# kibeomKim/Pytorch-DPPO

Hardware: AMD Instinct MI355X
Metric: env steps/sec (whole node), MuJoCo Humanoid-v2, 8 DPPO workers (higher is better)
Workload: dtype fp32_3xbf16; 1 GPU; model=reference actor-critic MLP (policy 376-100-100-17, value 376-500-100-1), global_batch=65536, seq_len=16, parallelism=dp1, env=Humanoid-v2, dppo_workers=1, workers_per_gpu=1, num_envs_per_gpu=4096, dist_backend=nccl, rccl_world_size=1, rollout_len=16, num_epoch=10, minibatch_rows=65536, overlap_rollout=False, per_head_kernels=True, grad_allreduce=none

## Files before the change

csrc/common.h:

```cpp
#pragma once
#include <hip/hip_runtime.h>
#include <hip/hip_fp8.h>
#include <stdint.h>

typedef __attribute__((ext_vector_type(4))) float f32x4;
typedef __attribute__((ext_vector_type(8))) __bf16 bf16x8;

#define DEV __device__ __forceinline__
typedef __attribute__((ext_vector_type(8))) float f32x8v;
DEV f32x4 ew_sub(const f32x4& a, const f32x4& b) { return a - b; }
DEV f32x8v ew_sub(const f32x8v& a, const f32x8v& b) { return a - b; }
DEV f32x8v ew_add(const f32x8v& a, const f32x8v& b) { return a + b; }
DEV f32x4 ew_mul(const f32x4& a, float s) { return a * s; }
DEV f32x4 ew_dtanh(const f32x4& a, const f32x4& h) { return a * (1.0f - h * h); }

enum { DT_F32 = 0, DT_BF16 = 1, DT_FP8 = 2, DT_S3 = 3 };

template <int DT> struct Prec;

template <> struct Prec<DT_F32> {
  using T = float;
  struct Frag { float4 lo, hi; };
  static constexpr int BYTES = 4;
  DEV static Frag load(const T* p) {
// ... 14 lines not shown
  DEV static T cvt(float x) { return x; }
  DEV static float tof(T x) { return x; }
  DEV static void put(T* b, size_t i, float x) { b[i] = x; }
  DEV static float get(const T* b, size_t i) { return b[i]; }
};

template <> struct Prec<DT_BF16> {
  using T = __bf16;
  using Frag = bf16x8;
  static constexpr int BYTES = 2;
  DEV static Frag load(const T* p) { return *reinterpret_cast<const bf16x8*>(p); }
  DEV static f32x4 mma(f32x4 c, const Frag& a, const Frag& b) {
    return __builtin_amdgcn_mfma_f32_16x16x32_bf16(a, b, c, 0, 0, 0);
  }
  DEV static T cvt(float x) { return (__bf16)x; }
  DEV static float tof(T x) { return (float)x; }
  DEV static void put(T* b, size_t i, float x) { b[i] = (__bf16)x; }
  DEV static float get(const T* b, size_t i) { return (float)b[i]; }
};

struct S3Slot { uint32_t raw; };
struct S3Frag { bf16x8 h, l; };
template <> struct Prec<DT_S3> {
  using T = S3Slot;
  using Frag = S3Frag;
  static constexpr int BYTES = 4;
  DEV static Frag load(const T* p) {
    const bf16x8* q = reinterpret_cast<const bf16x8*>(p);
    return Frag{q[0], q[1]};
  }
  DEV static f32x4 mma(f32x4 c, const Frag& a, const Frag& b) {
    c = __builtin_amdgcn_mfma_f32_16x16x32_bf16(a.l, b.h, c, 0, 0, 0);
    c = __builtin_amdgcn_mfma_f32_16x16x32_bf16(a.h, b.l, c, 0, 0, 0);
    return __builtin_amdgcn_mfma_f32_16x16x32_bf16(a.h, b.h, c, 0, 0, 0);
  }
  DEV static __bf16* hi_ptr(T* b, size_t i) { return reinterpret_cast<__bf16*>(b) + 2 * (i & ~size_t(7)) + (i & 7); }
  DEV static const __bf16* hi_ptr(const T* b, size_t i) {
    return reinterpret_cast<const __bf16*>(b) + 2 * (i & ~size_t(7)) + (i & 7);
  }
  DEV static void split(float x, __bf16& h, __bf16& l) {
    h = (__bf16)x;
    l = (__bf16)(x - (float)h);
  }
  DEV static void put(T* b, size_t i, float x) {
    __bf16* p = hi_ptr(b, i);
    split(x, p[0], p[8]);
  }
  DEV static float get(const T* b, size_t i) {
    const __bf16* p = hi_ptr(b, i);
    return (float)p[0] + (float)p[8];
  }
};
template <int DT> struct IsSplit { static constexpr bool value = DT == DT_S3; };

template <> struct Prec<DT_FP8> {
  using T = uint8_t;
  using Frag = long;
  static constexpr int BYTES = 1;
  DEV static Frag load(const T* p) { return *reinterpret_cast<const long*>(p); }
  DEV static f32x4 mma(f32x4 c, const Frag& a, const Frag& b) {
    return __builtin_amdgcn_mfma_f32_16x16x32_fp8_fp8(a, b, c, 0, 0, 0);
  }
  DEV static T cvt(float x) {
    __hip_fp8_e4m3 q(fminf(fmaxf(x, -448.f), 448.f));
    return *reinterpret_cast<uint8_t*>(&q);
  }
  DEV static float tof(T x) {
    __hip_fp8_e4m3 q;
    *reinterpret_cast<uint8_t*>(&q) = x;
    return float(q);
  }
  DEV static void put(T* b, size_t i, float x) { b[i] = cvt(x); }
  DEV static float get(const T* b, size_t i) { return tof(b[i]); }
};

__host__ __device__ inline size_t fm_index(int r, int c, int cols) {
  return ((size_t)(r >> 4) * (size_t)(cols >> 5) + (size_t)(c >> 5)) * 512u +
         (size_t)((((r & 15) + (((c & 31) >> 3) << 4)) << 3) + (c & 7));
}
__host__ __device__ inline size_t fm_frag(int rt, int ks, int cols, int lane) {
  return ((size_t)rt * (size_t)(cols >> 5) + (size_t)ks) * 512u + (size_t)lane * 8u;
}

template <typename V>
DEV void opnd_store(const V& v, V* p) {
  __builtin_nontemporal_store(v, p);
}

constexpr float Q8_SX = 64.f, Q8_SH = 256.f;
DEV uint32_t wave_umax(uint32_t v) {
#pragma unroll
  for (int o = 1; o < 64; o <<= 1) v = max(v, (uint32_t)__shfl_xor((int)v, o, 64));
  return v;
}
__host__ __device__ inline float q8_pow2(int e) {
  const uint32_t b = (uint32_t)(e + 127) << 23;
  float f;
  __builtin_memcpy(&f, &b, 4);
  return f;
}
__host__ __device__ inline int q8_exp(uint32_t amax_bits) {
  const int ex = (int)((amax_bits >> 23) & 0xffu);
  if (ex == 0 || ex == 255) return 0;
  const int e = 6 - (ex - 127);
  return e < -120 ? -120 : (e > 120 ? 120 : e);
}
DEV uint32_t q8_pack4(const f32x4& v, float s) {
  const float a = fminf(fmaxf(v[0] * s, -448.f), 448.f), b = fminf(fmaxf(v[1] * s, -448.f), 448.f);
  const float c = fminf(fmaxf(v[2] * s, -448.f), 448.f), d = fminf(fmaxf(v[3] * s, -448.f), 448.f);
  int w = __builtin_amdgcn_cvt_pk_fp8_f32(a, b, 0, false);
  return (uint32_t)__builtin_amdgcn_cvt_pk_fp8_f32(c, d, w, true);
}
DEV uint32_t q8_pack4u(const f32x4& v, float s) {
  int w = __builtin_amdgcn_cvt_pk_fp8_f32(v[0] * s, v[1] * s, 0, false);
  return (uint32_t)__builtin_amdgcn_cvt_pk_fp8_f32(v[2] * s, v[3] * s, w, true);
}
DEV float absmax4(const f32x4& v) { return fmaxf(fmaxf(fabsf(v[0]), fabsf(v[1])), fmaxf(fabsf(v[2]), fabsf(v[3]))); }

template <int DT> struct XStore { static constexpr int DTX = (DT == DT_FP8) ? DT_BF16 : DT; };

template <int DT> struct Lds {
  static constexpr int PAD = (DT == DT_FP8 ? 16 : 32) / Prec<DT>::BYTES;
  __host__ __device__ static constexpr int stride(int d) { return d + PAD; }
};

DEV float fast_tanh(float x) {
  const float e = __expf(-2.0f * fabsf(x));
  return copysignf((1.0f - e) * __builtin_amdgcn_rcpf(1.0f + e), x);
}

DEV uint32_t hash_u32(uint32_t x) {
  x ^= x >> 16; x *= 0x7FEB352Du; x ^= x >> 15; x *= 0x846CA68Bu; x ^= x >> 16;
  return x;
}
DEV uint32_t key_es(uint32_t base, uint32_t env, uint32_t step) { return hash_u32(hash_u32(env ^ base) ^ step); }
DEV uint32_t keyed(uint32_t base, uint32_t env, uint32_t step, uint32_t dim) {
  return hash_u32(key_es(base, env, step) ^ dim);
}
DEV float uniform01(uint32_t h) { return ((float)(h >> 8) + 0.5f) * (1.0f / 16777216.0f); }
DEV float2 gauss_pair(uint32_t kes, uint32_t p) {
  const float u1 = uniform01(hash_u32(kes ^ (2u * p)));
  const float u2 = uniform01(hash_u32(kes ^ (2u * p + 1u)));
  const float r = __builtin_sqrtf(-2.0f * 0.6931471805599453f * __builtin_amdgcn_logf(u1));
  return make_float2(r * __builtin_amdgcn_cosf(u2), r * __builtin_amdgcn_sinf(u2));
}
DEV float gauss(uint32_t base, uint32_t env, uint32_t step, uint32_t dim) {
  const float2 g = gauss_pair(key_es(base, env, step), dim >> 1);
  return (dim & 1u) ? g.y : g.x;
}

DEV void glds16(const void* g, void* lds) {
  __builtin_amdgcn_global_load_lds((const __attribute__((address_space(1))) void*)g,
                                   (__attribute__((address_space(3))) void*)lds, 16, 0, 0);
}

#define WAIT_VMCNT(n) __builtin_amdgcn_s_waitcnt((((n) & 15) | (7 << 4) | (15 << 8) | ((((n) >> 4) & 3) << 14)))

extern "C" void dppo_note_error(hipError_t e, const char* file, int line);

template <auto Kernel>
inline void set_max_lds_once(size_t bytes) {
  static size_t set = 0;
  if (bytes > set) {
    const hipError_t e = hipFuncSetAttribute(reinterpret_cast<const void*>(Kernel),
                                             hipFuncAttributeMaxDynamicSharedMemorySize, (int)bytes);
    if (e != hipSuccess) dppo_note_error(e, __FILE__, __LINE__);
    else set = bytes;
  }
}

#define HIP_CHECK_LAUNCH()                                          \
  do {                                                              \
    hipError_t e__ = hipGetLastError();                             \
    if (e__ != hipSuccess) dppo_note_error(e__, __FILE__, __LINE__); \
  } while (0)

__device__ __forceinline__ float slab_sum(const float* __restrict__ p, int nch, size_t st) {
  constexpr int B = 16;
  float s = 0.f;
  for (int c0 = 0; c0 < nch; c0 += B) {
    float x[B];
#pragma unroll
    for (int c = 0; c < B; ++c) x[c] = (c0 + c < nch) ? p[(size_t)(c0 + c) * st] : 0.f;
#pragma unroll
    for (int c = 0; c < B; ++c)
      if (c0 + c < nch) s += x[c];
  }
  return s;
}

__device__ __forceinline__ bool item_reduce(const float* __restrict__ part, int nprow, int npart,
                                            const int* __restrict__ red_col, int nitems, int b,
                                            float* red, float& out, int& j) {
  constexpr int RG = 256 / ITEM_IPB;
  const int tid = threadIdx.x, c = tid % ITEM_IPB, rg = tid / ITEM_IPB;
  j = ITEM_IPB * b + c;
  float s = 0.f;
  if (j < nitems && tid < 256) {
    const float* p = part + red_col[j];
    for (int r0 = rg; r0 < nprow; r0 += 16 * RG) {
      float x[16];
#pragma unroll
      for (int u = 0; u < 16; ++u) x[u] = (r0 + RG * u < nprow) ? p[(size_t)(r0 + RG * u) * npart] : 0.f;
#pragma unroll
      for (int u = 0; u < 16; ++u)
        if (r0 + RG * u < nprow) s += x[u];
    }
  }
  red[tid] = s;
  __syncthreads();
  if (tid < ITEM_IPB) {
    float o = red[tid];
#pragma unroll
    for (int g = 1; g < RG; ++g) o += red[g * ITEM_IPB + tid];
    out = o;
  }
  return tid < ITEM_IPB && j < nitems;
}
```

csrc/phead.hip:

```cpp
#include "t32.h"

namespace {

using namespace t32;

constexpr int PH_ROWS = 128;
constexpr int PH_WAVES = 4;
constexpr int PH_SB = 8 * 1024;
constexpr int PH_S = 3;
constexpr int PH_GL = 2;
constexpr int PH_XS = 3, PH_XB = 2048;
constexpr int PH_SCR = 48 * 1024;
constexpr int PH_RED = 64;
constexpr int PH_HP = 128 * 64 * 2;
constexpr int PH_DP = 128 * 32 * 2;

constexpr size_t ph_lds_bytes() {
  return (size_t)PH_S * PH_SB + PH_SCR + (PH_WAVES * PH_RED + 64) * sizeof(float);
}
static_assert(2 * ph_lds_bytes() <= 160 * 1024, "two policy workgroups per CU");
static_assert(PH_WAVES * PH_XS * PH_XB <= PH_SCR / 2 && PH_WAVES * 32 * 32 * 4 <= PH_SCR / 2 &&
              2 * PH_HP + 2 * PH_DP <= PH_SCR, "scratch: X rings | actions, then the dW staging");

DEV int ph_swz(int row) { return ((row >> 1) & 1) << 2; }

typedef __attribute__((ext_vector_type(4))) short s16x4;
DEV s16x4 tr4(const char* p) {
  s16x4 v;
  const unsigned addr = (unsigned)(size_t)(const __attribute__((address_space(3))) char*)(p);
  asm volatile("ds_read_b64_tr_b16 %0, %1" : "=v"(v) : "v"(addr));
  return v;
}
template <int DT>
DEV void ph_settle(typename VT<DT>::Frag (&fa)[2], typename VT<DT>::Frag (&fb)[2]) {
  if constexpr (DT == DT_S3) {
    asm volatile("s_waitcnt lgkmcnt(0)"
                 : "+v"(fa[0].h), "+v"(fa[0].l), "+v"(fa[1].h), "+v"(fa[1].l), "+v"(fb[0].h), "+v"(fb[0].l),
                   "+v"(fb[1].h), "+v"(fb[1].l));
  } else {
    asm volatile("s_waitcnt lgkmcnt(0)" : "+v"(fa[0]), "+v"(fa[1]), "+v"(fb[0]), "+v"(fb[1]));
  }
}
DEV bf16x8 cat8(s16x4 a0, s16x4 a1) {
  typedef __attribute__((ext_vector_type(8))) short s16x8;
  const s16x8 v{a0[0], a0[1], a0[2], a0[3], a1[0], a1[1], a1[2], a1[3]};
  return *reinterpret_cast<const bf16x8*>(&v);
}

DEV int ph_dim(int i, int h) { return (i & 3) + 8 * (i >> 2) + 4 * h; }

template <int DT, bool P2>
__global__ __launch_bounds__(PH_WAVES * 64, 2) void phead_kernel(MlpArgs a) {
  using V = VT<DT>;
  using Frag = typename V::Frag;
  constexpr bool S3 = DT == DT_S3;
  constexpr int EB = V::EB, KPS = V::KPS;
  constexpr int NS2 = S3 ? 7 : 4, NS3 = S3 ? 2 : 1, NG3 = S3 ? 2 : 1, NG2 = S3 ? 8 : 4;
  constexpr int KK2 = S3 ? 2 : 4;
  extern __shared__ __attribute__((aligned(16))) char smem[];
  const int tid = threadIdx.x, lane = tid & 63;
  const int wave = __builtin_amdgcn_readfirstlane(tid >> 6);
  const int h = lane >> 5, r = lane & 31;
  const int m0 = blockIdx.x * PH_ROWS;
  const int d0 = a.d_in[0];
  const int ns1 = (d0 >> 4) / KPS;
  const int e2 = ns1 + NS2, e3 = e2 + NS3, eg3 = e3 + NG3, ntot = eg3 + NG2;
  const int A = a.A;
  char* ring = smem;
  char* scr = smem + PH_S * PH_SB;
  char* xring = scr + wave * (PH_XS * PH_XB);
  float* red = reinterpret_cast<float*>(scr + PH_SCR);
  float* lsd = red + PH_WAVES * PH_RED;

  const int mr = m0 + 32 * wave + r;
  const bool valid = mr < a.M;
  const int rr = valid ? mr : m0;
  const int srow = a.idx ? a.idx[rr] : a.row0 + rr;
  const bool ref_loss = a.loss_kind != 0;
  float* acts = reinterpret_cast<float*>(scr + PH_SCR / 2) + wave * 32 * 32;
  {
    const float* arow = a.actions + (size_t)srow * A;
    for (int k = 0; 2 * k < A; ++k) {
      const int d = min(2 * k + h, A - 1);
      __builtin_amdgcn_global_load_lds((const __attribute__((address_space(1))) void*)(arow + d),
                                       (__attribute__((address_space(3))) void*)(acts + 64 * k), 4, 0, 0);
    }
  }
  float l_adv = a.adv[srow];
  float l_lpo = ref_loss ? 0.f : a.logp_old[srow];
  if (tid < 64) {
    const int j = tid & 31;
    lsd[tid] = tid < 32 ? (j < A ? a.log_std[j] : 0.f) : ((ref_loss && j < A) ? a.log_std_old[j] : 0.f);
  }

  const __amdgpu_buffer_rsrc_t rw = __builtin_amdgcn_make_buffer_rsrc(const_cast<void*>(a.W), (short)0, 0x7fffffff, 0x00020000);
  auto lane_off = [&](int c32, int d) __attribute__((always_inline)) -> unsigned {
    const int i = lane & 31;
    if constexpr (S3) return (unsigned)(((i >> 4) * c32 * 512 + ((i & 15) + 16 * d) * 8) * 4 + 16 * (lane >> 5));
    else return (unsigned)(((i >> 4) * c32 * 512 + ((i & 15) + 16 * (lane >> 5)) * 8) * 2);
  };
  const int c1 = d0 >> 5;
  const unsigned vo1[2] = {lane_off(c1, 0), lane_off(c1, 1)};
  const unsigned vo4[2] = {lane_off(4, 0), lane_off(4, 1)};
  const unsigned vog[2] = {lane_off(1, 0), lane_off(1, 1)};
  auto frag_u = [&](int t, int k16, int c32) __attribute__((always_inline)) {
    return t * 2 * c32 * 512 + (k16 >> 1) * 512 + (k16 & 1) * 256;
  };
  auto issue = [&](int st) __attribute__((always_inline)) {
    __attribute__((address_space(3))) char* dst =
        (__attribute__((address_space(3))) char*)(ring + (st % PH_S) * PH_SB);
#pragma unroll
    for (int i = 0; i < PH_GL; ++i) {
      const int I = PH_GL * wave + i;
      const int u = S3 ? I >> 1 : I, d = S3 ? (I & 1) : 0;
      const int tu = S3 ? u : (u & 3), ku = S3 ? 0 : (u >> 2);
      int off;
      unsigned voff;
      if (st < ns1) {
        off = a.off_w[0] + frag_u(tu, KPS * st + ku, c1);
        voff = vo1[d];
      } else if (st < e2) {
        off = a.off_w[1] + frag_u(tu, KPS * (st - ns1) + ku, 4);
        voff = vo4[d];
      } else if (st < e3) {
        off = a.off_w[2] + frag_u(0, S3 ? 4 * (st - e2) + u : u, 4);
        voff = vo4[d];
      } else if (st < eg3) {
        off = a.off_wt[2] + (S3 ? frag_u(2 * (st - e3) + (u & 1), u >> 1, 1) : frag_u(tu, ku, 1));
        voff = vog[d];
      } else {
        const int j = st - eg3, pass = j / (NG2 / 2), jj = j % (NG2 / 2);
        off = a.off_wt[1] + frag_u(2 * pass + (u & 1), KK2 * jj + (u >> 1), 4);
        voff = vo4[d];
      }
      __builtin_amdgcn_raw_ptr_buffer_load_lds(rw, dst + I * 1024, 16, voff, (unsigned)off * EB, 0, 0);
    }
  };
  const char* xrow = reinterpret_cast<const char*>(a.x_buf) + (size_t)srow * (size_t)d0 * EB;
  auto issue_x = [&](int st) __attribute__((always_inline)) {
    char* dx = xring + (st % PH_XS) * PH_XB;
#pragma unroll
    for (int e = 0; e < 2; ++e) {
      if constexpr (S3) glds16(xrow + (size_t)(16 * st + 8 * h) * 4 + 16 * e, dx + e * 1024);
      else glds16(xrow + (size_t)(16 * (2 * st + e) + 8 * h) * 2, dx + e * 1024);
    }
  };
  auto x_frag = [&](int st, int e) __attribute__((always_inline)) -> Frag {
    const char* xs = xring + (st % PH_XS) * PH_XB;
    if constexpr (S3) {
      return Frag{*reinterpret_cast<const bf16x8*>(xs + 16 * lane), *reinterpret_cast<const bf16x8*>(xs + 1024 + 16 * lane)};
    } else {
      return *reinterpret_cast<const bf16x8*>(xs + e * 1024 + 16 * lane);
    }
  };

  const __amdgpu_buffer_rsrc_t rs_x = __builtin_amdgcn_make_buffer_rsrc(a.xT, (short)0, 0x7fffffff, 0x00020000);
  const __amdgpu_buffer_rsrc_t rs_g1 = __builtin_amdgcn_make_buffer_rsrc(a.g1pT, (short)0, 0x7fffffff, 0x00020000);
  const __amdgpu_buffer_rsrc_t rs_h1 =
      __builtin_amdgcn_make_buffer_rsrc(P2 ? a.g1pT : a.h1pT, (short)0, 0x7fffffff, 0x00020000);
  const __amdgpu_buffer_rsrc_t rs_g2 =
      __builtin_amdgcn_make_buffer_rsrc(P2 ? a.g1pT : a.g2pT, (short)0, 0x7fffffff, 0x00020000);
  const unsigned vx = (unsigned)(mr * d0 + 8 * h) * EB, v128 = (unsigned)(mr * 128 + 8 * h) * EB;
  const bool write_x = a.xT_ready == 0;
  const int xst = write_x ? 2 : 0;

  asm volatile("s_waitcnt vmcnt(0)" : "+v"(l_adv), "+v"(l_lpo)::"memory");
  static_assert(PH_S == 3 && PH_XS == 3, "the wait counts below are written for 3-stage rings");
  issue_x(0);
  issue_x(1);
  issue(0);
  issue(1);

  f32x16 acc1[4], acc2[4];
#pragma unroll
  for (int t = 0; t < 4; ++t) acc1[t] = acc2[t] = f32x16{};

  auto sync = [&](int younger) __attribute__((always_inline)) {
    asm volatile("" ::: "memory");
    wait_vm_rt(younger);
    asm volatile("s_waitcnt lgkmcnt(0)" ::: "memory");
    __builtin_amdgcn_s_barrier();
    asm volatile("" ::: "memory");
  };
  VmTrack vt(ns1 == 3 ? 2 + PH_GL + xst : 2 + PH_GL + 2 * xst, xst);
  constexpr int SP = S3 ? 2 : 1;
  auto sync_t = [&](int st) __attribute__((always_inline)) {
    sync(vt.younger());
    const bool refill = st + 2 < ntot;
    if (refill) issue(st + 2);
    vt.advance(refill ? PH_GL : 0);
  };
  auto sync_late = [&](int st) __attribute__((always_inline)) {
    sync_t(st);
    return ring + (st % PH_S) * PH_SB;
  };
  auto sto = [&](__amdgpu_buffer_rsrc_t rs, unsigned vrow, unsigned fsoff, const Frag& f) __attribute__((always_inline)) {
    st_op<DT>(rs, vrow, fsoff, f);
    vt.add(SP);
  };
// ... 424 lines not shown
```

csrc/wgrad.hip:

```cpp
#include "kernels.h"
#include "mlp_core.h"

namespace {

constexpr int WG_WAVES = 8;

template <int DT>
constexpr int wgrad_frag_bytes() { return DT == DT_FP8 ? 2048 : 512 * Prec<DT>::BYTES; }
template <int DT>
constexpr int wgrad_step_rows() { return DT == DT_FP8 ? 128 : 32; }
typedef __attribute__((ext_vector_type(8))) int i32x8;

__host__ __device__ inline int wgrad_swz(int row) { return (((row >> 1) & 1) << 1) | (((row >> 3) & 1) << 2); }

DEV unsigned rm_off(int f, int sub, int lane, int FB) {
  const int li = lane & 15, g = lane >> 4;
  const int row = 8 * g + 4 * sub + (li >> 2), col = 16 * (f & 3) + 4 * (li & 3);
  return (unsigned)((f & ~3) * FB + row * 128 + (((col >> 3) ^ wgrad_swz(row)) << 4) + (col & 7) * 2);
}
__host__ __device__ inline int wgrad_swz16(int row) { return ((row & 3) << 2) | ((row >> 3) & 3); }
DEV unsigned rm_off_s3(int f, int sub, int part, int lane, int FB) {
  const int li = lane & 15, g = lane >> 4;
  const int row = 8 * g + 4 * sub + (li >> 2), col = 16 * (f & 3) + 4 * (li & 3);
  const int pos = ((col >> 3) * 2 + part) ^ wgrad_swz16(row);
  return (unsigned)((f & ~3) * FB + row * 256 + pos * 16 + (col & 7) * 2);
}
template <int DT>
DEV typename Prec<DT>::Frag rm_frag_at(const char* st, const unsigned (&o)[4]) {
  typedef __attribute__((ext_vector_type(4))) short s16x4;
  typedef __attribute__((ext_vector_type(8))) short s16x8;
  auto rd = [&](unsigned off) __attribute__((always_inline)) {
    return __builtin_amdgcn_ds_read_tr16_b64_v4i16((__attribute__((address_space(3))) s16x4*)(st + off));
  };
  auto cat = [&](s16x4 a0, s16x4 a1) __attribute__((always_inline)) {
    const s16x8 v{a0[0], a0[1], a0[2], a0[3], a1[0], a1[1], a1[2], a1[3]};
    return *reinterpret_cast<const bf16x8*>(&v);
  };
  if constexpr (IsSplit<DT>::value) {
    return S3Frag{cat(rd(o[0]), rd(o[1])), cat(rd(o[2]), rd(o[3]))};
  } else {
    return cat(rd(o[0]), rd(o[1]));
  }
}

template <int DT, int QW>
struct WgCfg {
  static constexpr int SLOTS = QW == 1 ? 24 : 40;
  static constexpr int S = DT == DT_BF16 ? 4 : (QW == 1 ? 3 : 2);
};
template <int DT, bool WIDE>
constexpr size_t wgrad_lds_bytes() {
  constexpr size_t one = (size_t)WgCfg<DT, 1>::S * WgCfg<DT, 1>::SLOTS * wgrad_frag_bytes<DT>();
  constexpr size_t two = (size_t)WgCfg<DT, 2>::S * WgCfg<DT, 2>::SLOTS * wgrad_frag_bytes<DT>();
  return WIDE && two > one ? two : one;
}
static_assert(wgrad_lds_bytes<DT_S3, true>() <= 160 * 1024 && wgrad_lds_bytes<DT_BF16, true>() <= 160 * 1024, "wgrad LDS");

template <int DT, int QW, int C>
DEV void wgrad_lds_body(const WgradArgs& a, const WgradTask& tk, char* smem) {
  using P = Prec<DT>;
  using T = typename P::T;
  using Frag = typename P::Frag;
  constexpr int FB = wgrad_frag_bytes<DT>();
  constexpr int NI = FB / 1024;
  constexpr int S = WgCfg<DT, QW>::S;
  constexpr int SB = WgCfg<DT, QW>::SLOTS * FB;
  static_assert(QW == 1 || DT == DT_S3 || DT == DT_BF16, "two quadrants per wave: split-bf16 / bf16");
  static_assert(C * WG_WAVES <= WgCfg<DT, QW>::SLOTS, "slots");
  const int tid = threadIdx.x, lane = tid & 63;
  const int wave = __builtin_amdgcn_readfirstlane(tid >> 6);
  const char* g = reinterpret_cast<const char*>(a.gT[tk.layer]);
  const char* x = reinterpret_cast<const char*>(a.xT[tk.layer]);
  const int nk = (tk.m1 - tk.m0) / wgrad_step_rows<DT>();
  const int ks0 = tk.m0 >> 5;
  const int NF = 4 * tk.nq, F = NF + 4 * tk.kq;
  const char* srcp[C][NI];
  size_t kstride[C];
  int dst[C];
#pragma unroll
  for (int q = 0; q < C; ++q) {
    const int f = wave * C + q;
    const int ff = f < F ? f : f % F;
    const bool gs = ff < NF;
    const int fl = gs ? ff : ff - NF;
    const int feat0 = (gs ? tk.n0 : tk.k0) + 16 * fl;
    const int rm = (DT == DT_S3 || DT == DT_BF16) ? (gs ? a.g_rm[tk.layer] : a.x_rm[tk.layer]) : 0;
    const char* ob = gs ? g : x;
    if (rm == 0) {
      const char* src = ob + fm_frag(feat0 >> 4, ks0, a.ld, 0) * sizeof(T);
#pragma unroll
      for (int hh = 0; hh < NI; ++hh)
        srcp[q][hh] = src + (IsSplit<DT>::value ? (size_t)hh * 1024 + (lane & 31) * 32 + (lane >> 5) * 16
                                                 : (size_t)hh * 1024 + lane * 16);
      kstride[q] = FB;
    } else {
      const int sq = fl & 3, f0 = feat0 - 16 * sq;
#pragma unroll
      for (int hh = 0; hh < NI; ++hh) {
        const int n = NI * sq + hh;
        if constexpr (IsSplit<DT>::value) {
          const int row = 4 * n + (lane >> 4);
          const int c = (lane & 15) ^ wgrad_swz16(row);
          srcp[q][hh] = ob + ((size_t)(tk.m0 + row) * rm + f0) * sizeof(T) + 16 * c;
        } else {
          const int row = 8 * n + (lane >> 3);
          const int c = (lane & 7) ^ wgrad_swz(row);
          srcp[q][hh] = ob + ((size_t)(tk.m0 + row) * rm + f0 + 8 * c) * sizeof(T);
        }
      }
      kstride[q] = (size_t)32 * rm * sizeof(T);
    }
    dst[q] = f * FB;
  }
  auto issue = [&](int k) {
    const int kk = min(k, nk - 1);
    char* st = smem + (k % S) * SB;
#pragma unroll
    for (int q = 0; q < C; ++q)
#pragma unroll
      for (int h = 0; h < NI; ++h) glds16(srcp[q][h] + (size_t)kk * kstride[q], st + dst[q] + h * 1024);
  };
  uint32_t q8v = 0;
  if constexpr (DT == DT_FP8) q8v = a.q8_rd[(a.q8_t[tk.layer] * Q8_SUB + lane) * Q8_LINE];
  const int nqw = QW == 1 ? tk.nq : tk.nq >> 1;
  const bool active = wave < nqw * tk.kq;
  constexpr bool RMOK = DT == DT_S3 || DT == DT_BF16;
  const bool g_rm = RMOK && a.g_rm[tk.layer] != 0, x_rm = RMOK && a.x_rm[tk.layer] != 0;
  const int wn = wave / tk.kq, wk = wave - (wave / tk.kq) * tk.kq;
  const unsigned fmo = IsSplit<DT>::value ? (unsigned)((lane >> 5) * 1024 + (lane & 31) * 16)
                                          : (unsigned)(lane * 8 * (int)sizeof(T));
  unsigned pat[4][4];
#pragma unroll
  for (int i = 0; i < 4; ++i) {
    pat[i][0] = pat[i][1] = pat[i][2] = pat[i][3] = 0;
    if constexpr (IsSplit<DT>::value) {
      for (int j = 0; j < 4; ++j) pat[i][j] = rm_off_s3(i, j & 1, j >> 1, lane, FB);
    } else if constexpr (RMOK) {
      pat[i][0] = rm_off(i, 0, lane, FB);
      pat[i][1] = rm_off(i, 1, lane, FB);
    }
  }
  auto frag = [&](const char* st, int slot, bool rm, int i) __attribute__((always_inline)) -> Frag {
    const char* qb = st + slot * FB;
    if constexpr (RMOK)
      if (rm) return rm_frag_at<DT>(qb, pat[i]);
    const char* b = qb + fmo + i * FB;
    if constexpr (IsSplit<DT>::value) {
      return Frag{*reinterpret_cast<const bf16x8*>(b), *reinterpret_cast<const bf16x8*>(b + 512)};
    } else {
      return P::load(reinterpret_cast<const T*>(b));
    }
  };
  f32x4 acc[QW][4][4];
#pragma unroll
  for (int u = 0; u < QW; ++u)
#pragma unroll
    for (int i = 0; i < 4; ++i)
#pragma unroll
      for (int j = 0; j < 4; ++j) acc[u][i][j] = f32x4{0.f, 0.f, 0.f, 0.f};
#pragma unroll
  for (int s = 0; s < S - 1; ++s) issue(s);
  for (int k = 0; k < nk; ++k) {
    WAIT_VMCNT(C * NI * (S - 2));
    __builtin_amdgcn_s_barrier();
    constexpr bool LATE = DT != DT_FP8;
    if (!LATE || !active) issue(k + S - 1);
    if (active) {
      const char* st = smem + (k % S) * SB;
      if constexpr (DT == DT_FP8) {
        auto rd = [&](int f) {
          const char* p = st + f * FB + lane * 8;
          const long x0 = *reinterpret_cast<const long*>(p), x1 = *reinterpret_cast<const long*>(p + 512);
          const long x2 = *reinterpret_cast<const long*>(p + 1024), x3 = *reinterpret_cast<const long*>(p + 1536);
          return i32x8{(int)x0, (int)(x0 >> 32), (int)x1, (int)(x1 >> 32), (int)x2, (int)(x2 >> 32), (int)x3,
                       (int)(x3 >> 32)};
        };
        i32x8 a8[4], b8[4];
#pragma unroll
        for (int i = 0; i < 4; ++i) {
          a8[i] = rd(wn * 4 + i);
          b8[i] = rd(NF + wk * 4 + i);
        }

#pragma unroll
        for (int i = 0; i < 4; ++i)
#pragma unroll
          for (int j = 0; j < 4; ++j)
            acc[0][i][j] = __builtin_amdgcn_mfma_scale_f32_16x16x128_f8f6f4(a8[i], b8[j], acc[0][i][j], 0, 0, 0, 127, 0, 127);
        continue;
      }
      Frag af[4], bf[4];
#pragma unroll
      for (int i = 0; i < 4; ++i) {
        af[i] = frag(st, 4 * wn, g_rm, i);
        bf[i] = frag(st, NF + 4 * wk, x_rm, i);
      }
      if constexpr (LATE) issue(k + S - 1);
#pragma unroll
      for (int i = 0; i < 4; ++i)
#pragma unroll
        for (int j = 0; j < 4; ++j) acc[0][i][j] = P::mma(acc[0][i][j], af[i], bf[j]);
      if constexpr (QW == 2) {
#pragma unroll
        for (int i = 0; i < 4; ++i) af[i] = frag(st, 4 * (wn + nqw), g_rm, i);
#pragma unroll
        for (int i = 0; i < 4; ++i)
#pragma unroll
          for (int j = 0; j < 4; ++j) acc[QW - 1][i][j] = P::mma(acc[QW - 1][i][j], af[i], bf[j]);
      }
    }
  }
  WAIT_VMCNT(0);
  if (!active) return;
  const int KE = tk.kq * 64;
  float* out = a.slab + tk.slab;
  if constexpr (DT == DT_FP8) {
    const float inv = q8_pow2(-q8_exp(wave_umax(q8v))) / a.q8_xs[tk.layer];
#pragma unroll
    for (int i = 0; i < 4; ++i)
#pragma unroll
      for (int j = 0; j < 4; ++j) acc[0][i][j] *= inv;
  }
  const int col = wk * 64 + (lane & 15);
#pragma unroll
  for (int u = 0; u < QW; ++u) {
    const int rbase = (wn + u * nqw) * 64 + (lane >> 4) * 4;
#pragma unroll
    for (int i = 0; i < 4; ++i)
#pragma unroll
      for (int j = 0; j < 4; ++j)
#pragma unroll
        for (int q = 0; q < 4; ++q) out[(rbase + 16 * i + q) * KE + col + 16 * j] = acc[u][i][j][q];
  }
}

template <int DT, bool WIDE>
__global__ __launch_bounds__(WG_WAVES * 64) void wgrad_kernel(WgradArgs a) {
  extern __shared__ __attribute__((aligned(16))) char smem[];
  const WgradTask tk = a.tasks[blockIdx.x];
  const int F = 4 * (tk.nq + tk.kq);
  if constexpr (WIDE) {
    if (tk.nq * tk.kq > WG_WAVES) {
      if (F <= 4 * WG_WAVES) wgrad_lds_body<DT, 2, 4>(a, tk, smem);
      else wgrad_lds_body<DT, 2, 5>(a, tk, smem);
      return;
    }
  }
  if (F <= 2 * WG_WAVES) wgrad_lds_body<DT, 1, 2>(a, tk, smem);
  else wgrad_lds_body<DT, 1, 3>(a, tk, smem);
}

template <int DT, bool WIDE>
void launch_wgrad_lds(const WgradArgs& a, hipStream_t s) {
  const size_t lds = wgrad_lds_bytes<DT, WIDE>();
  set_max_lds_once<wgrad_kernel<DT, WIDE>>(lds);
  hipLaunchKernelGGL((wgrad_kernel<DT, WIDE>), dim3(a.ntasks), dim3(WG_WAVES * 64), lds, s, a);
}

__global__ __launch_bounds__(256) void grad_gather_kernel(const float* __restrict__ slab,
                                                          const int* __restrict__ src_off,
                                                          const int* __restrict__ src_meta,
                                                          const float* __restrict__ part,
                                                          int nblk, int npart, const int* __restrict__ red_col,
                                                          const int* __restrict__ red_dst, int nitems,
                                                          float scale, float* __restrict__ grad, SlabRuns runs,
                                                          float* __restrict__ loss_out) {
  const int nrb = item_blocks(nitems);
  if ((int)blockIdx.x < nrb) {
    __shared__ float red[256];
    float tot = 0.f;
    int j;
    if (item_reduce(part, nblk, npart, red_col, nitems, blockIdx.x, red, tot, j)) {
      const int d = red_dst[j];
      if (d >= 0) grad[d] = tot * scale;
      else loss_out[-1 - d] = tot;
    }
    return;
  }
  const int nb = gridDim.x - nrb;
  for (int j = (blockIdx.x - nrb) * 256 + threadIdx.x; j < runs.total; j += nb * 256) {
    const int i = runs.flat(j);
    const int mt = src_meta[i];
    const int o = src_off[i];
    const int nch = mt >> 5;
    const size_t st = (size_t)(mt & 31) << 12;
    const float s = slab_sum(slab + o, nch, st);
    grad[i] = s * scale;
  }
}

}

extern "C" int wgrad_task_ok(int dt, int nq, int kq) {
  if (nq < 1 || kq < 1) return 0;
  if (nq * kq <= WG_WAVES) return nq + kq <= 6;
  return (dt == DT_S3 || dt == DT_BF16) && nq * kq <= 2 * WG_WAVES && nq % 2 == 0 && nq + kq <= 10;
}

extern "C" void launch_wgrad(int dt, const WgradArgs& a, hipStream_t s) {
  if (a.ntasks <= 0) return;
  if (dt == DT_F32) launch_wgrad_lds<DT_F32, false>(a, s);
  else if (dt == DT_FP8) launch_wgrad_lds<DT_FP8, false>(a, s);
  else if (dt == DT_S3) {
    if (a.wide) launch_wgrad_lds<DT_S3, true>(a, s);
    else launch_wgrad_lds<DT_S3, false>(a, s);
  } else {
    if (a.wide) launch_wgrad_lds<DT_BF16, true>(a, s);
    else launch_wgrad_lds<DT_BF16, false>(a, s);
  }
  HIP_CHECK_LAUNCH();
}

extern "C" void launch_grad_gather(const float* slab, const int* src_off, const int* src_meta, const float* part,
                                   int nblk, int npart, const int* red_col, const int* red_dst, int nitems,
                                   float scale, float* grad, const SlabRuns& runs, float* loss_out, hipStream_t s) {
  int grid = (runs.total + 255) / 256;
  if (grid > 2048) grid = 2048;
  if (grid < 1) grid = 1;
  grid += item_blocks(nitems);
  hipLaunchKernelGGL(grad_gather_kernel, dim3(grid), dim3(256), 0, s, slab, src_off, src_meta, part, nblk, npart,
                     red_col, red_dst, nitems, scale, grad, runs, loss_out);
  HIP_CHECK_LAUNCH();
}
```

pytorch_dppo_amd/ops/_build.py:

```python
from __future__ import annotations

import concurrent.futures as cf
import hashlib
import os
import subprocess
import sys
import sysconfig

ROOT = os.path.dirname(os.path.dirname(os.path.dirname(os.path.abspath(__file__))))
CSRC = os.path.join(ROOT, "csrc")
BUILD = os.path.join(ROOT, "build")
OUT_DIR = os.path.dirname(os.path.abspath(__file__))
EXT_NAME = "_dppo_hip"
ARCH = os.environ.get("DPPO_OFFLOAD_ARCH", "gfx950")
HIPCC = os.environ.get("HIPCC", "/opt/rocm/bin/hipcc")
DEVICE_SRCS = ["rollout.hip", "eval.hip", "mlp.hip", "mlp_head.hip", "phead.hip", "wgrad.hip", "optim.hip", "obs.hip"]
HOST_SRCS = ["bindings.cpp", "comm.cpp"]
HEADERS = ["common.h", "mlp_core.h", "kernels.h", "t32.h"]


def ext_path(variant: str = "") -> str:
    name = EXT_NAME + (f"_{variant}" if variant else "")
    return os.path.join(OUT_DIR, name + sysconfig.get_config_var("EXT_SUFFIX"))


def _torch_flags(ext_name: str = EXT_NAME):
    import torch
    from torch.utils import cpp_extension as ce
    inc = ce.include_paths(device_type="cuda")
    libdirs = ce.library_paths(device_type="cuda")
    abi = int(torch._C._GLIBCXX_USE_CXX11_ABI)
    cflags = [f"-I{p}" for p in inc] + [f"-I{sysconfig.get_paths()['include']}",
                                         f"-D_GLIBCXX_USE_CXX11_ABI={abi}",
                                         f"-DTORCH_EXTENSION_NAME={ext_name}",
                                         "-DTORCH_API_INCLUDE_EXTENSION_H", "-DUSE_ROCM=1"]
    ldflags = [f"-L{p}" for p in libdirs] + [f"-Wl,-rpath,{p}" for p in libdirs] + [
        "-lc10", "-ltorch", "-ltorch_cpu", "-ltorch_python", "-lc10_hip", "-ltorch_hip",
        "-lrccl"]
    return cflags, ldflags


def _digest(paths, extra: str) -> str:
    h = hashlib.sha256(extra.encode())
    for p in paths:
        with open(p, "rb") as f:
            h.update(f.read())
    return h.hexdigest()[:16]


def _compile(src: str, cflags, verbose: bool, csrc: str = CSRC, extra=()) -> str:
    srcp = os.path.join(csrc, src)
    deps = [srcp] + [os.path.join(csrc, h) for h in HEADERS]
    base = ["-O3", "-std=c++17", "-fPIC", f"--offload-arch={ARCH}", "-Wno-unused-result",
            "-mllvm", "-amdgpu-mfma-vgpr-form"]
    base += os.environ.get("DPPO_EXTRA_CFLAGS", "").split() + list(extra)
    flags = base + cflags
    key = _digest(deps, " ".join(flags))
    obj = os.path.join(BUILD, f"{os.path.splitext(src)[0]}-{key}.o")
    if os.path.exists(obj):
        return obj
    cmd = [HIPCC] + flags + ["-c", srcp, "-o", obj]
    if verbose:
        print(" ".join(cmd), flush=True)
    r = subprocess.run(cmd, capture_output=True, text=True)
    if r.returncode != 0:
        raise RuntimeError(f"hipcc failed for {src}:\n{r.stderr[-6000:]}")
    return obj


def build(verbose: bool = False, force: bool = False, variant: str = "", csrc: str = CSRC, defines=()) -> str:
    os.makedirs(BUILD, exist_ok=True)
    tcflags, ldflags = _torch_flags(EXT_NAME + (f"_{variant}" if variant else ""))
    jobs = [(s, []) for s in DEVICE_SRCS] + [(s, tcflags) for s in HOST_SRCS]
    with cf.ThreadPoolExecutor(max_workers=min(8, os.cpu_count() or 4)) as ex:
        extra = [f"-D{d}" for d in defines]
        objs = list(ex.map(lambda j: _compile(j[0], j[1], verbose, csrc, extra), jobs))
    out = ext_path(variant)
    key = hashlib.sha256((" ".join(os.path.basename(o) for o in objs) + " "
                          + " ".join(ldflags)).encode()).hexdigest()[:16]
    stamp = out + ".stamp"
    if not force and os.path.exists(out) and os.path.exists(stamp) and open(stamp).read() == key:
        return out
    tmp = out + ".tmp.so"
    cmd = [HIPCC, "-shared", "-fPIC", f"--offload-arch={ARCH}"] + objs + ldflags + ["-o", tmp]
    if verbose:
        print(" ".join(cmd), flush=True)
    r = subprocess.run(cmd, capture_output=True, text=True)
    if r.returncode != 0:
        raise RuntimeError(f"link failed:\n{r.stderr[-6000:]}")
    os.replace(tmp, out)
    with open(stamp, "w") as f:
        f.write(key)
    return out


if __name__ == "__main__":
    args = sys.argv[1:]
    var = args[args.index("--variant") + 1] if "--variant" in args else ""
    src = args[args.index("--src") + 1] if "--src" in args else CSRC
    defs = args[args.index("--define") + 1].split(",") if "--define" in args else []
    p = build(verbose="-v" in args, force="--force" in args, variant=var, csrc=src, defines=defs)
    print(p)
```

Before: 15.93 million env_steps/s.

## Specialize wgrad on operand layout and add half-stage LDS ring for split-bf16

The weight-gradient kernel is now instantiated per combination of row-major or feature-major operand layout, so the runtime branch inside the inner loop is gone. LDS fragment reads now use inline asm with immediate offsets, are issued before the next async global-to-LDS refill, and are drained with one explicit lgkmcnt wait. For split-bf16 with two quadrants per wave, a new five-unit half-stage ring refills half-tiles at a finer grain to deepen prefetch within the LDS budget. The rewritten addressing and wait counts add risk of ordering or correctness errors, and having more template variants increases code size.

```diff
diff --git a/csrc/common.h b/csrc/common.h
--- a/csrc/common.h
+++ b/csrc/common.h
@@ -190,6 +190,36 @@
 DEV void glds16(const void* g, void* lds) {
   __builtin_amdgcn_global_load_lds((const __attribute__((address_space(1))) void*)g,
                                    (__attribute__((address_space(3))) void*)lds, 16, 0, 0);
+}
+
+typedef __attribute__((ext_vector_type(4))) short s16x4;
+DEV unsigned lds_addr(const void* p) {
+  return (unsigned)(size_t)(const __attribute__((address_space(3))) char*)(p);
+}
+DEV s16x4 tr4(const char* p) {
+  s16x4 v;
+  const unsigned addr = lds_addr(p);
+  asm volatile("ds_read_b64_tr_b16 %0, %1" : "=v"(v) : "v"(addr));
+  return v;
+}
+template <int OFF>
+DEV s16x4 tr4_at(unsigned addr) {
+  static_assert(OFF >= 0 && OFF < 65536, "ds offset field");
+  s16x4 v;
+  asm volatile("ds_read_b64_tr_b16 %0, %1 offset:%2" : "=v"(v) : "v"(addr), "i"(OFF));
+  return v;
+}
+template <int OFF>
+DEV bf16x8 lds_rd16_at(unsigned addr) {
+  static_assert(OFF >= 0 && OFF < 65536, "ds offset field");
+  bf16x8 v;
+  asm volatile("ds_read_b128 %0, %1 offset:%2" : "=v"(v) : "v"(addr), "i"(OFF));
+  return v;
+}
+DEV bf16x8 cat8(s16x4 a0, s16x4 a1) {
+  typedef __attribute__((ext_vector_type(8))) short s16x8;
+  const s16x8 v{a0[0], a0[1], a0[2], a0[3], a1[0], a1[1], a1[2], a1[3]};
+  return *reinterpret_cast<const bf16x8*>(&v);
 }
 
 #define WAIT_VMCNT(n) __builtin_amdgcn_s_waitcnt((((n) & 15) | (7 << 4) | (15 << 8) | ((((n) >> 4) & 3) << 14)))
diff --git a/csrc/phead.hip b/csrc/phead.hip
--- a/csrc/phead.hip
+++ b/csrc/phead.hip
@@ -24,13 +24,6 @@
 
 DEV int ph_swz(int row) { return ((row >> 1) & 1) << 2; }
 
-typedef __attribute__((ext_vector_type(4))) short s16x4;
-DEV s16x4 tr4(const char* p) {
-  s16x4 v;
-  const unsigned addr = (unsigned)(size_t)(const __attribute__((address_space(3))) char*)(p);
-  asm volatile("ds_read_b64_tr_b16 %0, %1" : "=v"(v) : "v"(addr));
-  return v;
-}
 template <int DT>
 DEV void ph_settle(typename VT<DT>::Frag (&fa)[2], typename VT<DT>::Frag (&fb)[2]) {
   if constexpr (DT == DT_S3) {
@@ -40,11 +33,6 @@
   } else {
     asm volatile("s_waitcnt lgkmcnt(0)" : "+v"(fa[0]), "+v"(fa[1]), "+v"(fb[0]), "+v"(fb[1]));
   }
-}
-DEV bf16x8 cat8(s16x4 a0, s16x4 a1) {
-  typedef __attribute__((ext_vector_type(8))) short s16x8;
-  const s16x8 v{a0[0], a0[1], a0[2], a0[3], a1[0], a1[1], a1[2], a1[3]};
-  return *reinterpret_cast<const bf16x8*>(&v);
 }
 
 DEV int ph_dim(int i, int h) { return (i & 3) + 8 * (i >> 2) + 4 * h; }
diff --git a/csrc/wgrad.hip b/csrc/wgrad.hip
--- a/csrc/wgrad.hip
+++ b/csrc/wgrad.hip
@@ -1,3 +1,5 @@
+#include <type_traits>
+
 #include "kernels.h"
 #include "mlp_core.h"
 
@@ -19,44 +21,85 @@
   return (unsigned)((f & ~3) * FB + row * 128 + (((col >> 3) ^ wgrad_swz(row)) << 4) + (col & 7) * 2);
 }
 __host__ __device__ inline int wgrad_swz16(int row) { return ((row & 3) << 2) | ((row >> 3) & 3); }
-DEV unsigned rm_off_s3(int f, int sub, int part, int lane, int FB) {
+DEV unsigned rm_off_s3(int f, int sub, int part, int lane, int FB, int rmask = 31) {
   const int li = lane & 15, g = lane >> 4;
   const int row = 8 * g + 4 * sub + (li >> 2), col = 16 * (f & 3) + 4 * (li & 3);
   const int pos = ((col >> 3) * 2 + part) ^ wgrad_swz16(row);
-  return (unsigned)((f & ~3) * FB + row * 256 + pos * 16 + (col & 7) * 2);
-}
-template <int DT>
-DEV typename Prec<DT>::Frag rm_frag_at(const char* st, const unsigned (&o)[4]) {
-  typedef __attribute__((ext_vector_type(4))) short s16x4;
-  typedef __attribute__((ext_vector_type(8))) short s16x8;
-  auto rd = [&](unsigned off) __attribute__((always_inline)) {
-    return __builtin_amdgcn_ds_read_tr16_b64_v4i16((__attribute__((address_space(3))) s16x4*)(st + off));
-  };
-  auto cat = [&](s16x4 a0, s16x4 a1) __attribute__((always_inline)) {
-    const s16x8 v{a0[0], a0[1], a0[2], a0[3], a1[0], a1[1], a1[2], a1[3]};
-    return *reinterpret_cast<const bf16x8*>(&v);
-  };
+  return (unsigned)((f & ~3) * FB + (row & rmask) * 256 + pos * 16 + (col & 7) * 2);
+}
+template <int DT, bool RM>
+struct WgRaw {
+  using Piece = std::conditional_t<RM, s16x4, bf16x8>;
+  static constexpr int NP = (IsSplit<DT>::value ? 2 : 1) * (RM ? 2 : 1);
+  Piece p[NP];
+};
+template <int DT, bool RM, int FBS, int I>
+DEV void wg_read(WgRaw<DT, RM>& r, unsigned qb, unsigned fmo, const unsigned (&rmo)[4][2]) {
+  constexpr bool SP = IsSplit<DT>::value;
+  if constexpr (RM) {
+    constexpr int SUB = 4 * (SP ? 256 : 128);
+    r.p[0] = tr4_at<0>(qb + rmo[I][0]);
+    r.p[1] = tr4_at<SUB>(qb + rmo[I][0]);
+    if constexpr (SP) {
+      r.p[2] = tr4_at<0>(qb + rmo[I][1]);
+      r.p[3] = tr4_at<SUB>(qb + rmo[I][1]);
+    }
+  } else {
+    r.p[0] = lds_rd16_at<I * FBS>(qb + fmo);
+    if constexpr (SP) r.p[1] = lds_rd16_at<I * FBS + 512>(qb + fmo);
+  }
+}
+template <int DT, bool RM, int FBS>
+DEV void wg_read4(WgRaw<DT, RM> (&r)[4], unsigned qb, unsigned fmo, const unsigned (&rmo)[4][2]) {
+  wg_read<DT, RM, FBS, 0>(r[0], qb, fmo, rmo);
+  wg_read<DT, RM, FBS, 1>(r[1], qb, fmo, rmo);
+  wg_read<DT, RM, FBS, 2>(r[2], qb, fmo, rmo);
+  wg_read<DT, RM, FBS, 3>(r[3], qb, fmo, rmo);
+}
+DEV void wg_lgkm0() { asm volatile("s_waitcnt lgkmcnt(0)"); }
+template <int DT, bool RM>
+DEV void wg_pin(WgRaw<DT, RM>& r) {
+  if constexpr (WgRaw<DT, RM>::NP == 4) asm volatile("" : "+v"(r.p[0]), "+v"(r.p[1]), "+v"(r.p[2]), "+v"(r.p[3]));
+  else if constexpr (WgRaw<DT, RM>::NP == 2) asm volatile("" : "+v"(r.p[0]), "+v"(r.p[1]));
+  else asm volatile("" : "+v"(r.p[0]));
+}
+template <int DT, bool RM>
+DEV typename Prec<DT>::Frag wg_frag(const WgRaw<DT, RM>& r) {
   if constexpr (IsSplit<DT>::value) {
-    return S3Frag{cat(rd(o[0]), rd(o[1])), cat(rd(o[2]), rd(o[3]))};
+    if constexpr (RM) return S3Frag{cat8(r.p[0], r.p[1]), cat8(r.p[2], r.p[3])};
+    else return S3Frag{r.p[0], r.p[1]};
   } else {
-    return cat(rd(o[0]), rd(o[1]));
-  }
-}
-
+    if constexpr (RM) return cat8(r.p[0], r.p[1]);
+    else return r.p[0];
+  }
+}
+
+#ifndef WGRAD_HALF_RING
+#define WGRAD_HALF_RING 1
+#endif
 template <int DT, int QW>
 struct WgCfg {
   static constexpr int SLOTS = QW == 1 ? 24 : 40;
   static constexpr int S = DT == DT_BF16 ? 4 : (QW == 1 ? 3 : 2);
 };
+struct WgHalf {
+  static constexpr int SLOTS = 32, UNITS = 5, UB = SLOTS * 1024;
+};
+template <int DT, int QW, int C>
+constexpr bool wgrad_half_ring() { return WGRAD_HALF_RING && DT == DT_S3 && QW == 2 && C == 4; }
 template <int DT, bool WIDE>
 constexpr size_t wgrad_lds_bytes() {
   constexpr size_t one = (size_t)WgCfg<DT, 1>::S * WgCfg<DT, 1>::SLOTS * wgrad_frag_bytes<DT>();
   constexpr size_t two = (size_t)WgCfg<DT, 2>::S * WgCfg<DT, 2>::SLOTS * wgrad_frag_bytes<DT>();
-  return WIDE && two > one ? two : one;
-}
-static_assert(wgrad_lds_bytes<DT_S3, true>() <= 160 * 1024 && wgrad_lds_bytes<DT_BF16, true>() <= 160 * 1024, "wgrad LDS");
-
-template <int DT, int QW, int C>
+  constexpr size_t half = DT == DT_S3 ? (size_t)WgHalf::UNITS * WgHalf::UB : 0;
+  constexpr size_t wide = two > half ? two : half;
+  return WIDE && wide > one ? wide : one;
+}
+static_assert(wgrad_lds_bytes<DT_S3, true>() <= 160 * 1024 && wgrad_lds_bytes<DT_BF16, true>() <= 160 * 1024 &&
+              wgrad_lds_bytes<DT_F32, false>() <= 160 * 1024 && wgrad_lds_bytes<DT_FP8, false>() <= 160 * 1024 &&
+              (size_t)WgHalf::UNITS * WgHalf::UB <= 160 * 1024, "every wgrad ring fits the CU's 160 KiB of LDS");
+
+template <int DT, int QW, int C, bool G_RM, bool X_RM>
 DEV void wgrad_lds_body(const WgradArgs& a, const WgradTask& tk, char* smem) {
   using P = Prec<DT>;
   using T = typename P::T;
@@ -65,8 +108,12 @@
   constexpr int NI = FB / 1024;
   constexpr int S = WgCfg<DT, QW>::S;
   constexpr int SB = WgCfg<DT, QW>::SLOTS * FB;
+  constexpr bool RMOK = DT == DT_S3 || DT == DT_BF16;
+  constexpr bool HALF = wgrad_half_ring<DT, QW, C>();
   static_assert(QW == 1 || DT == DT_S3 || DT == DT_BF16, "two quadrants per wave: split-bf16 / bf16");
   static_assert(C * WG_WAVES <= WgCfg<DT, QW>::SLOTS, "slots");
+  static_assert(RMOK || (!G_RM && !X_RM), "row-major operands: split-bf16 / bf16");
+  static_assert(!HALF || (C * WG_WAVES == WgHalf::SLOTS && NI == 2), "half-stage ring: a quadrant per wave");
   const int tid = threadIdx.x, lane = tid & 63;
   const int wave = __builtin_amdgcn_readfirstlane(tid >> 6);
   const char* g = reinterpret_cast<const char*>(a.gT[tk.layer]);
@@ -84,7 +131,7 @@
     const bool gs = ff < NF;
     const int fl = gs ? ff : ff - NF;
     const int feat0 = (gs ? tk.n0 : tk.k0) + 16 * fl;
-    const int rm = (DT == DT_S3 || DT == DT_BF16) ? (gs ? a.g_rm[tk.layer] : a.x_rm[tk.layer]) : 0;
+    const int rm = gs ? (G_RM ? a.g_rm[tk.layer] : 0) : (X_RM ? a.x_rm[tk.layer] : 0);
     const char* ob = gs ? g : x;
     if (rm == 0) {
       const char* src = ob + fm_frag(feat0 >> 4, ks0, a.ld, 0) * sizeof(T);
@@ -120,37 +167,42 @@
 #pragma unroll
       for (int h = 0; h < NI; ++h) glds16(srcp[q][h] + (size_t)kk * kstride[q], st + dst[q] + h * 1024);
   };
+  const char* usrc[2][4];
+  if constexpr (HALF) {
+    const bool rmw = (wave * C < F ? wave * C : (wave * C) % F) < NF ? G_RM : X_RM;
+#pragma unroll
+    for (int h = 0; h < 2; ++h)
+#pragma unroll
+      for (int j = 0; j < 4; ++j) usrc[h][j] = rmw ? srcp[2 * h + (j >> 1)][j & 1] : srcp[j][h];
+  }
+  auto issue_half = [&](auto H, int k, int pos) __attribute__((always_inline)) {
+    const int kk = min(k, nk - 1);
+    char* ub = smem + pos * WgHalf::UB + wave * 4096;
+#pragma unroll
+    for (int j = 0; j < 4; ++j) glds16(usrc[H.value][j] + (size_t)kk * kstride[0], ub + j * 1024);
+  };
+  auto mod5 = [](int u) { return u >= WgHalf::UNITS ? u - WgHalf::UNITS : u; };
   uint32_t q8v = 0;
   if constexpr (DT == DT_FP8) q8v = a.q8_rd[(a.q8_t[tk.layer] * Q8_SUB + lane) * Q8_LINE];
   const int nqw = QW == 1 ? tk.nq : tk.nq >> 1;
   const bool active = wave < nqw * tk.kq;
-  constexpr bool RMOK = DT == DT_S3 || DT == DT_BF16;
-  const bool g_rm = RMOK && a.g_rm[tk.layer] != 0, x_rm = RMOK && a.x_rm[tk.layer] != 0;
   const int wn = wave / tk.kq, wk = wave - (wave / tk.kq) * tk.kq;
-  const unsigned fmo = IsSplit<DT>::value ? (unsigned)((lane >> 5) * 1024 + (lane & 31) * 16)
-                                          : (unsigned)(lane * 8 * (int)sizeof(T));
-  unsigned pat[4][4];
+  constexpr int FBS = HALF ? 1024 : FB;
+  const unsigned fmo = HALF ? (unsigned)((lane & 31) * 16)
+                            : IsSplit<DT>::value ? (unsigned)((lane >> 5) * 1024 + (lane & 31) * 16)
+                                                 : (unsigned)(lane * 8 * (int)sizeof(T));
+  unsigned rmo[4][2];
 #pragma unroll
   for (int i = 0; i < 4; ++i) {
-    pat[i][0] = pat[i][1] = pat[i][2] = pat[i][3] = 0;
+    rmo[i][0] = rmo[i][1] = 0;
     if constexpr (IsSplit<DT>::value) {
-      for (int j = 0; j < 4; ++j) pat[i][j] = rm_off_s3(i, j & 1, j >> 1, lane, FB);
+      rmo[i][0] = rm_off_s3(i, 0, 0, lane, FB, HALF ? 15 : 31);
+      rmo[i][1] = rm_off_s3(i, 0, 1, lane, FB, HALF ? 15 : 31);
     } else if constexpr (RMOK) {
-      pat[i][0] = rm_off(i, 0, lane, FB);
-      pat[i][1] = rm_off(i, 1, lane, FB);
-    }
-  }
-  auto frag = [&](const char* st, int slot, bool rm, int i) __attribute__((always_inline)) -> Frag {
-    const char* qb = st + slot * FB;
-    if constexpr (RMOK)
-      if (rm) return rm_frag_at<DT>(qb, pat[i]);
-    const char* b = qb + fmo + i * FB;
-    if constexpr (IsSplit<DT>::value) {
-      return Frag{*reinterpret_cast<const bf16x8*>(b), *reinterpret_cast<const bf16x8*>(b + 512)};
-    } else {
-      return P::load(reinterpret_cast<const T*>(b));
-    }
-  };
+      rmo[i][0] = rm_off(i, 0, lane, FB);
+    }
+  }
+  const unsigned lds0 = lds_addr(smem);
   f32x4 acc[QW][4][4];
 #pragma unroll
   for (int u = 0; u < QW; ++u)
@@ -158,16 +210,33 @@
     for (int i = 0; i < 4; ++i)
 #pragma unroll
       for (int j = 0; j < 4; ++j) acc[u][i][j] = f32x4{0.f, 0.f, 0.f, 0.f};
-#pragma unroll
-  for (int s = 0; s < S - 1; ++s) issue(s);
+  int p5 = 0;
+  if constexpr (HALF) {
+    issue_half(std::integral_constant<int, 0>{}, 0, 0);
+    issue_half(std::integral_constant<int, 1>{}, 0, 1);
+    issue_half(std::integral_constant<int, 0>{}, 1, 2);
+  } else {
+#pragma unroll
+    for (int s = 0; s < S - 1; ++s) issue(s);
+  }
   for (int k = 0; k < nk; ++k) {
-    WAIT_VMCNT(C * NI * (S - 2));
+    if constexpr (HALF) WAIT_VMCNT(4);
+    else WAIT_VMCNT(C * NI * (S - 2));
     __builtin_amdgcn_s_barrier();
     constexpr bool LATE = DT != DT_FP8;
-    if (!LATE || !active) issue(k + S - 1);
+    auto refill = [&]() __attribute__((always_inline)) {
+      if constexpr (HALF) {
+        issue_half(std::integral_constant<int, 1>{}, k + 1, mod5(p5 + 3));
+        issue_half(std::integral_constant<int, 0>{}, k + 2, mod5(p5 + 4));
+      } else {
+        issue(k + S - 1);
+      }
+    };
+    if (!LATE || !active) refill();
     if (active) {
-      const char* st = smem + (k % S) * SB;
       if constexpr (DT == DT_FP8) {
+        static_assert(DT != DT_FP8 || QW == 1, "the e4m3 scale epilogue covers acc[0] only");
+        const char* st = smem + (k % S) * SB;
         auto rd = [&](int f) {
           const char* p = st + f * FB + lane * 8;
           const long x0 = *reinterpret_cast<const long*>(p), x1 = *reinterpret_cast<const long*>(p + 512);
@@ -188,27 +257,60 @@
           for (int j = 0; j < 4; ++j)
             acc[0][i][j] = __builtin_amdgcn_mfma_scale_f32_16x16x128_f8f6f4(a8[i], b8[j], acc[0][i][j], 0, 0, 0, 127, 0, 127);
         continue;
+      } else if constexpr (!RMOK) {
+        const char* st = smem + (k % S) * SB;
+        Frag af[4], bf[4];
+#pragma unroll
+        for (int i = 0; i < 4; ++i) {
+          af[i] = P::load(reinterpret_cast<const T*>(st + (4 * wn + i) * FB + fmo));
+          bf[i] = P::load(reinterpret_cast<const T*>(st + (NF + 4 * wk + i) * FB + fmo));
+        }
+        issue(k + S - 1);
+#pragma unroll
+        for (int i = 0; i < 4; ++i)
+#pragma unroll
+          for (int j = 0; j < 4; ++j) acc[0][i][j] = P::mma(acc[0][i][j], af[i], bf[j]);
+      } else {
+        unsigned sa;
+        if constexpr (HALF) sa = lds0 + (unsigned)((lane >> 5) ? mod5(p5 + 1) : p5) * WgHalf::UB;
+        else sa = lds0 + (unsigned)((k % S) * SB);
+        WgRaw<DT, G_RM> ar[4];
+        WgRaw<DT, X_RM> br[4];
+        wg_read4<DT, G_RM, FBS>(ar, sa + 4 * wn * FBS, fmo, rmo);
+        wg_read4<DT, X_RM, FBS>(br, sa + (NF + 4 * wk) * FBS, fmo, rmo);
+        refill();
+        wg_lgkm0();
+#pragma unroll
+        for (int i = 0; i < 4; ++i) wg_pin(ar[i]);
+#pragma unroll
+        for (int i = 0; i < 4; ++i) wg_pin(br[i]);
+        __builtin_amdgcn_sched_barrier(0);
+        Frag af[4], bf[4];
+#pragma unroll
+        for (int i = 0; i < 4; ++i) {
+          af[i] = wg_frag(ar[i]);
+          bf[i] = wg_frag(br[i]);
+        }
+#pragma unroll
+        for (int i = 0; i < 4; ++i)
+#pragma unroll
+          for (int j = 0; j < 4; ++j) acc[0][i][j] = P::mma(acc[0][i][j], af[i], bf[j]);
+        if constexpr (QW == 2) {
+          wg_read4<DT, G_RM, FBS>(ar, sa + 4 * (wn + nqw) * FBS, fmo, rmo);
+          wg_lgkm0();
+#pragma unroll
+          for (int i = 0; i < 4; ++i) wg_pin(ar[i]);
+          __builtin_amdgcn_sched_barrier(0);
+#pragma unroll
+          for (int i = 0; i < 4; ++i) af[i] = wg_frag(ar[i]);
+#pragma unroll
+          for (int i = 0; i < 4; ++i)
+#pragma unroll
+            for (int j = 0; j < 4; ++j) acc[QW - 1][i][j] = P::mma(acc[QW - 1][i][j], af[i], bf[j]);
+        }
       }
-      Frag af[4], bf[4];
-#pragma unroll
-      for (int i = 0; i < 4; ++i) {
-        af[i] = frag(st, 4 * wn, g_rm, i);
-        bf[i] = frag(st, NF + 4 * wk, x_rm, i);
-      }
-      if constexpr (LATE) issue(k + S - 1);
-#pragma unroll
-      for (int i = 0; i < 4; ++i)
-#pragma unroll
-        for (int j = 0; j < 4; ++j) acc[0][i][j] = P::mma(acc[0][i][j], af[i], bf[j]);
-      if constexpr (QW == 2) {
-#pragma unroll
-        for (int i = 0; i < 4; ++i) af[i] = frag(st, 4 * (wn + nqw), g_rm, i);
-#pragma unroll
-        for (int i = 0; i < 4; ++i)
-#pragma unroll
-          for (int j = 0; j < 4; ++j) acc[QW - 1][i][j] = P::mma(acc[QW - 1][i][j], af[i], bf[j]);
-      }
-    }
+    }
+    if constexpr (HALF) p5 = mod5(p5 + 2);
   }
   WAIT_VMCNT(0);
   if (!active) return;
@@ -231,6 +333,22 @@
       for (int j = 0; j < 4; ++j)
 #pragma unroll
         for (int q = 0; q < 4; ++q) out[(rbase + 16 * i + q) * KE + col + 16 * j] = acc[u][i][j][q];
+  }
+}
+
+template <int DT, int QW, int C>
+DEV void wgrad_by_layout(const WgradArgs& a, const WgradTask& tk, char* smem) {
+  if constexpr (DT == DT_S3 || DT == DT_BF16) {
+    const bool g_rm = a.g_rm[tk.layer] != 0, x_rm = a.x_rm[tk.layer] != 0;
+    if (g_rm) {
+      if (x_rm) wgrad_lds_body<DT, QW, C, true, true>(a, tk, smem);
+      else wgrad_lds_body<DT, QW, C, true, false>(a, tk, smem);
+    } else {
+      if (x_rm) wgrad_lds_body<DT, QW, C, false, true>(a, tk, smem);
+      else wgrad_lds_body<DT, QW, C, false, false>(a, tk, smem);
+    }
+  } else {
+    wgrad_lds_body<DT, QW, C, false, false>(a, tk, smem);
   }
 }
 
@@ -241,13 +359,13 @@
   const int F = 4 * (tk.nq + tk.kq);
   if constexpr (WIDE) {
     if (tk.nq * tk.kq > WG_WAVES) {
-      if (F <= 4 * WG_WAVES) wgrad_lds_body<DT, 2, 4>(a, tk, smem);
-      else wgrad_lds_body<DT, 2, 5>(a, tk, smem);
+      if (F <= 4 * WG_WAVES) wgrad_by_layout<DT, 2, 4>(a, tk, smem);
+      else wgrad_by_layout<DT, 2, 5>(a, tk, smem);
       return;
     }
   }
-  if (F <= 2 * WG_WAVES) wgrad_lds_body<DT, 1, 2>(a, tk, smem);
-  else wgrad_lds_body<DT, 1, 3>(a, tk, smem);
+  if (F <= 2 * WG_WAVES) wgrad_by_layout<DT, 1, 2>(a, tk, smem);
+  else wgrad_by_layout<DT, 1, 3>(a, tk, smem);
 }
 
 template <int DT, bool WIDE>
diff --git a/pytorch_dppo_amd/ops/_build.py b/pytorch_dppo_amd/ops/_build.py
--- a/pytorch_dppo_amd/ops/_build.py
+++ b/pytorch_dppo_amd/ops/_build.py
@@ -48,13 +48,16 @@
     return h.hexdigest()[:16]
 
 
+def device_flags(extra=()) -> list:
+    base = ["-O3", "-std=c++17", "-fPIC", f"--offload-arch={ARCH}", "-Wno-unused-result",
+            "-mllvm", "-amdgpu-mfma-vgpr-form"]
+    return base + os.environ.get("DPPO_EXTRA_CFLAGS", "").split() + list(extra)
+
+
 def _compile(src: str, cflags, verbose: bool, csrc: str = CSRC, extra=()) -> str:
     srcp = os.path.join(csrc, src)
     deps = [srcp] + [os.path.join(csrc, h) for h in HEADERS]
-    base = ["-O3", "-std=c++17", "-fPIC", f"--offload-arch={ARCH}", "-Wno-unused-result",
-            "-mllvm", "-amdgpu-mfma-vgpr-form"]
-    base += os.environ.get("DPPO_EXTRA_CFLAGS", "").split() + list(extra)
-    flags = base + cflags
+    flags = device_flags(extra) + cflags
     key = _digest(deps, " ".join(flags))
     obj = os.path.join(BUILD, f"{os.path.splitext(src)[0]}-{key}.o")
     if os.path.exists(obj):
```

Result: faster. 16.23 million env_steps/s, median of 6 (+1.9%).
